# winddori2002/DEX-TTS

Hardware: AMD Instinct MI355X
Metric: mel-frames/s at n_timesteps=50, 80-ch mel (sampler only); RTF (higher is better)
Workload: dtype bf16; 1 GPU; gedex_b1: gedex_lj B=1/GPU T=512 n_timesteps=50 (BASELINE.json configs[1]); global_batch=1, frames=512, hipgraph=False, parallelism=1 GPU

## Files before the change

dex_tts_amd/csrc/conv3x3_bf16.hip:

```cpp
#include "kernels.h"
#include <cstdlib>
#include <cstdio>
#include "lp_util.h"
#include "kernels_lp.h"
#include "conv_gn.h"

namespace dex {
namespace DEX_LP_NS {

typedef float f32x16 __attribute__((ext_vector_type(16)));
typedef unsigned short u16;
typedef unsigned u32x4 __attribute__((ext_vector_type(4)));

__device__ __forceinline__ float cv_mish(float x) {
    const float e = __expf(fminf(x, 20.f));
    const float n = e * (e + 2.f);
    return x * (n * __builtin_amdgcn_rcpf(n + 2.f));
}

template <int NT, int COUT>
__device__ __forceinline__ void cv_epilogue(const Conv3P& p, f32x16 (&acc)[NT], int b, int ho, int w0, int nbase, int lane, int tid,
                                            long long* gnred) {
    const int i = lane & 31, hh = lane >> 5;
    constexpr int cpg = COUT / 8;
    if (p.gn_stats) { if (tid < 16) gnred[tid] = 0; __syncthreads(); }
    const bool full = ho < p.H && w0 + 32 <= p.W;
    const long ybase = (long)b * p.H * p.W * COUT + ((long)ho * p.W + w0 + 4 * hh) * COUT + nbase + i;
    float* yl = p.Y + ybase;
    u16* yh = reinterpret_cast<u16*>(p.Y) + ybase;
    const bool yb = p.y_bf16 != 0;
#pragma unroll
    for (int t = 0; t < NT; ++t) {
        const int n = nbase + t * 32 + i;
        const float bias = p.bias[n];
        float gs = 0.f, gss = 0.f;
        if (full && yb) {
            const bool odd = (lane & 1) != 0;
            u16* yp = yh + (odd ? 16 * COUT - 1 : 0) + t * 32;
#pragma unroll
            for (int r = 0; r < 16; ++r) { const float v = acc[t][r] + bias; gs += v; gss = fmaf(v, v, gss); }
#pragma unroll
            for (int j = 0; j < 8; ++j) {
                const float lo_r = acc[t][j] + bias, hi_r = acc[t][8 + j] + bias;
                const float recv = lane_xor1(odd ? lo_r : hi_r);
                const float mine = odd ? hi_r : lo_r;
                const unsigned pk = odd ? pack2_lp(recv, mine) : pack2_lp(mine, recv);
                *reinterpret_cast<unsigned*>(yp + ((j & 3) + 8 * (j >> 2)) * COUT) = pk;
            }
        } else if (full) {
            const bool odd = (lane & 1) != 0;
            float* yp = yl + (odd ? 16 * COUT - 1 : 0) + t * 32;
#pragma unroll
            for (int r = 0; r < 16; ++r) { const float v = acc[t][r] + bias; gs += v; gss = fmaf(v, v, gss); }
#pragma unroll
            for (int j = 0; j < 8; ++j) {
                const float lo_r = acc[t][j] + bias, hi_r = acc[t][8 + j] + bias;
                const float recv = lane_xor1(odd ? lo_r : hi_r);
                const float mine = odd ? hi_r : lo_r;
                *reinterpret_cast<float2*>(yp + ((j & 3) + 8 * (j >> 2)) * COUT) = odd ? make_float2(recv, mine) : make_float2(mine, recv);
            }
        } else {
#pragma unroll
            for (int r = 0; r < 16; ++r) {
                const int wo = w0 + (r & 3) + 8 * (r >> 2) + 4 * hh;
                const bool ok = ho < p.H && wo < p.W;
                const float v = acc[t][r] + bias;
                const float vs = ok ? v : 0.f;
                gs += vs; gss = fmaf(vs, vs, gss);
                if (ok) {
                    if (yb) yh[((r & 3) + 8 * (r >> 2)) * COUT + t * 32] = lp_bits(v);
                    else yl[((r & 3) + 8 * (r >> 2)) * COUT + t * 32] = v;
                }
            }
        }
        if (p.gn_stats) {
            for (int o = 1; o < cpg; o <<= 1) { gs += __shfl_xor(gs, o); gss += __shfl_xor(gss, o); }
            gs += __shfl_xor(gs, 32); gss += __shfl_xor(gss, 32);
            if (hh == 0 && (i & (cpg - 1)) == 0) {
                const double inv_n = 1.0 / ((double)p.H * p.W * cpg);
                gn_add(&gnred[(n / cpg) * 2], gn_fix(gs, inv_n)); gn_add(&gnred[(n / cpg) * 2 + 1], gn_fix(gss, inv_n));
            }
        }
    }
    if (p.gn_stats) {
        __syncthreads();
        if (tid < 16) {
            const long long v = gnred[tid];
            if (v != 0) {
                const int slot = (blockIdx.x + blockIdx.y * gridDim.x) % GN_SLOTS;
                gn_add(p.gn_stats + (((long)b * 8 + (tid >> 1)) * GN_SLOTS + slot) * 2 + (tid & 1), v);
            }
        }
    }
}

template <int NT, int COUT>
__device__ __forceinline__ void cv_res_store(const Conv3P& p, const f32x16 (&accr)[NT], int b, int ho, int w0, int nb, int lane) {
    const int i = lane & 31, hh = lane >> 5;
    float* yl = p.res_y + ((long)b * p.H * p.W + (long)ho * p.W + w0 + 4 * hh) * COUT + nb + i;
    const bool rfull = ho < p.H && w0 + 32 <= p.W;
    const bool odd = (lane & 1) != 0;
#pragma unroll
    for (int t = 0; t < NT; ++t) {
        const float bias = p.res_b[nb + t * 32 + i];
        if (rfull) {
            float* yp = yl + (odd ? 16 * COUT - 1 : 0) + t * 32;
#pragma unroll
            for (int j = 0; j < 8; ++j) {
                const float lo_r = accr[t][j] + bias, hi_r = accr[t][8 + j] + bias;
                const float recv = lane_xor1(odd ? lo_r : hi_r);
                const float mine = odd ? hi_r : lo_r;
                *reinterpret_cast<float2*>(yp + ((j & 3) + 8 * (j >> 2)) * COUT) = odd ? make_float2(recv, mine) : make_float2(mine, recv);
            }
        } else {
#pragma unroll
            for (int r = 0; r < 16; ++r) {
                const int wo = w0 + (r & 3) + 8 * (r >> 2) + 4 * hh;
                if (ho < p.H && wo < p.W) yl[((r & 3) + 8 * (r >> 2)) * COUT + t * 32] = accr[t][r] + bias;
            }
        }
    }
}

template <int CC, int COUT, int NSL, int TH, bool PRO2 = false, bool RES = false, bool XB = false, int NW = 4, bool RW = false>
__global__ __launch_bounds__(64 * NW) void conv3x3_lp_kernel(const Conv3P p) {
    constexpr int PW = 34, PH = TH + 2;
    constexpr int LDP = CC + 8;
    constexpr int WN = NW / TH;
    constexpr int NTHR = 64 * NW;
    constexpr int NT = NSL / 32 / WN;
    constexpr int NSLICE = COUT / NSL;
    constexpr int ITEMS = PH * PW * (CC / 8);
    constexpr int NI = (ITEMS + NTHR - 1) / NTHR;
    constexpr int WITEMS = NSL * CC / 8;
    constexpr int WPT = (WITEMS + NTHR - 1) / NTHR;
    constexpr bool WFULL = WITEMS % NTHR == 0;
    constexpr int RING = CC == 128 ? (PRO2 ? 1 : 2) : 3;
    constexpr int NPASS = RW ? 1
                        : TH == 5 ? (CC == 128 ? (PRO2 ? 6 : 3) : (PRO2 ? 3 : XB ? 1 : 2))
                                  : CC == 128 ? (TH == 8 ? (PRO2 ? 8 : 4) : (PRO2 ? 5 : 2)) : (PRO2 ? 3 : 1);
    constexpr int NIP = (NI + NPASS - 1) / NPASS;
    constexpr int RWI = 9 * WITEMS;
    constexpr int RWPT = (RWI + NTHR - 1) / NTHR;
    constexpr int RWB = (RWPT + NPASS - 1) / NPASS;
#ifdef DEX_LP_WSPLIT
    constexpr int NTAP = 18;
#else
    constexpr int NTAP = 9;
#endif
    static_assert(NT >= 1 && WPT >= 1 && NW % TH == 0 && NTHR % (CC / 8) == 0, "tile");
    static_assert(!RW || NTAP == 9, "the resident schedule holds nine taps");
    extern __shared__ __attribute__((aligned(16))) u16 smem[];
    u16* patch = smem;
    u16* wbuf = smem + PH * PW * LDP;
    u16* rbuf = wbuf + (RW ? 9 : 2) * NSL * LDP;
    __shared__ long long gnred[16];
    constexpr int COEF_N = (TH == 8) ? 128 : 256;
    __shared__ __attribute__((aligned(16))) float coef[3][COEF_N];

    const int tid = threadIdx.x, lane = tid & 63, wave = tid >> 6;
    const int i = lane & 31, hh = lane >> 5;
    const int wrow = wave % TH, wcol = wave / TH;
#ifdef DEX_TIMING
    long long tk[8] = {0, 0, 0, 0, 0, 0, 0, 0};
    const long long tk0 = __builtin_readcyclecounter();
    long long tlast = tk0;
#define CSTAMP(k) do { const long long now_ = __builtin_readcyclecounter(); tk[k] += now_ - tlast; tlast = now_; } while (0)
#else
#define CSTAMP(k) do {} while (0)
#endif
    const int xs = p.skip_dead ? (int)((blockIdx.x + blockIdx.y + blockIdx.z) % gridDim.x) : (int)blockIdx.x;
    const int w0 = xs * 32, h0 = blockIdx.y * TH;
    const int b = blockIdx.z / NSLICE, slice = blockIdx.z % NSLICE;
    const int step = p.step + b * p.row_bstride;
    const float* X = p.X + (long)b * p.H * p.W * p.ldx + p.x_coff;
    const u16* Xh = reinterpret_cast<const u16*>(p.X) + (long)b * p.H * p.W * p.ldx + p.x_coff;
    const float* mrow = p.mask + (long)b * p.mask_bstride;
    const int K = 9 * p.Cin;
    const u16* Wg = reinterpret_cast<const u16*>(p.Wbf) + (long)slice * NSL * K;
    const bool pro = p.pro_stats != nullptr;
    if constexpr (!PRO2) {
        if (p.skip_dead) {
            const int wi = w0 - 1 + (lane < 34 ? lane : 33);
            const float mv = (unsigned)wi < (unsigned)p.W ? mrow[wi * p.mask_ws] : 0.f;
            if (__builtin_amdgcn_ballot_w64(mv != 0.f) == 0) {
                f32x16 zacc[NT];
#pragma unroll
                for (int t = 0; t < NT; ++t)
#pragma unroll
                    for (int r = 0; r < 16; ++r) zacc[t][r] = 0.f;
                if constexpr (RES) cv_res_store<NT, COUT>(p, zacc, b, h0 + wrow, w0, slice * NSL + wcol * NT * 32, lane);
                cv_epilogue<NT, COUT>(p, zacc, b, h0 + wrow, w0, slice * NSL + wcol * NT * 32, lane, tid, gnred);
                return;
            }
        }
    }

    f32x16 acc[NT];
#pragma unroll
    for (int t = 0; t < NT; ++t)
#pragma unroll
        for (int r = 0; r < 16; ++r) acc[t][r] = 0.f;

    f32x16 accr[RES ? NT : 1];
    if constexpr (RES) {
#pragma unroll
        for (int t = 0; t < NT; ++t)
#pragma unroll
            for (int r = 0; r < 16; ++r) accr[t][r] = 0.f;
    }
    int wofs[WPT], wlds[WPT];
    bool wok[WPT];
#pragma unroll
    for (int j = 0; j < WPT; ++j) {
        const int it = tid + NTHR * j;
        const int n = it / (CC / 8), c8 = (it % (CC / 8)) * 8;
        wofs[j] = n * K + c8;
        wlds[j] = n * LDP + c8;
        wok[j] = WFULL || it < WITEMS;
    }
    const int pc8 = (tid % (CC / 8)) * 8;

    CvGnLoads gnl{};
    if (pro) gnl = cv_gn_issue(p, b, tid, step);
    const int nchunk = RW ? 1 : p.Cin / CC;
    for (int ch = 0; ch < nchunk; ++ch) {
        const int cbase = ch * CC;
        u32x4 w0r[WPT], wr[RING][WPT], rwr[RES ? WPT : 1];
#ifdef DEX_LP_WSPLIT
        u32x4 rwl[RES ? WPT : 1];
#define WS_TAPOFS(t) ((long)((t) % 9) * p.Cin + ((t) >= 9 ? p.w_lo_off : 0L))
#else
#define WS_TAPOFS(t) ((long)(t) * p.Cin)
#endif
        float4 sc0, sc1, sh0, sh1, t0, t1;
#pragma unroll
        for (int ps = 0; ps < NPASS; ++ps) {
            float4 pf0[NIP], pf1[XB ? 1 : NIP], rf0[PRO2 ? NIP : 1], rf1[PRO2 ? NIP : 1];
            float pmk[NIP];
            bool pin[NIP];
#pragma unroll
            for (int q = 0; q < NIP; ++q) {
                const int it = min(tid + NTHR * (ps * NIP + q), ITEMS - 1);
                const int px = it / (CC / 8);
                const int pw = px % PW, ph = px / PW;
                const int hi = h0 + ph - 1, wi = w0 + pw - 1;
                const bool inb = (unsigned)hi < (unsigned)p.H && (unsigned)wi < (unsigned)p.W;
                const int hc = inb ? hi : 0, wc = inb ? wi : 0;
                if constexpr (XB) {
                    pf0[q] = *reinterpret_cast<const float4*>(Xh + ((long)hc * p.W + wc) * p.ldx + cbase + pc8);
                } else {
                    const float* src = X + ((long)hc * p.W + wc) * p.ldx + cbase + pc8;
                    pf0[q] = *reinterpret_cast<const float4*>(src);
                    pf1[q] = *reinterpret_cast<const float4*>(src + 4);
                }
                if constexpr (PRO2) {
                    const float* rs = p.pro_res + ((long)b * p.H * p.W + (long)hc * p.W + wc) * p.Cin + cbase + pc8;
                    rf0[q] = *reinterpret_cast<const float4*>(rs);
                    rf1[q] = *reinterpret_cast<const float4*>(rs + 4);
                }
                const float mk = mrow[wc * p.mask_ws];
                pmk[q] = inb ? mk : 0.f;
                pin[q] = inb;
            }
            u32x4 rwv[RW ? RWB : 1];
            if constexpr (RW) {
#pragma unroll
                for (int j = 0; j < RWB; ++j) {
                    const int it = tid + NTHR * (ps * RWB + j);
                    if (ps * RWB + j < RWPT && (RWI % NTHR == 0 || it < RWI)) {
                        const int r = it % WITEMS;
                        rwv[j] = *reinterpret_cast<const u32x4*>(Wg + (r / (CC / 8)) * K + (it / WITEMS) * p.Cin + (r % (CC / 8)) * 8);
                    }
                }
            }
            if (ps == 0) {
                if constexpr (RES) {
                    const u16* Rg = reinterpret_cast<const u16*>(p.res_w) + (long)slice * NSL * p.Cin;
#pragma unroll
                    for (int j = 0; j < WPT; ++j) {
                        const int it = tid + NTHR * j;
                        if (!wok[j]) continue;
                        rwr[j] = *reinterpret_cast<const u32x4*>(Rg + (long)(it / (CC / 8)) * p.Cin + cbase + (it % (CC / 8)) * 8);
#ifdef DEX_LP_WSPLIT
                        rwl[j] = *reinterpret_cast<const u32x4*>(Rg + p.res_lo_off + (long)(it / (CC / 8)) * p.Cin + cbase + (it % (CC / 8)) * 8);
#endif
                    }
                }
                if constexpr (!RW) {
#pragma unroll
                    for (int j = 0; j < WPT; ++j) if (wok[j]) w0r[j] = *reinterpret_cast<const u32x4*>(Wg + wofs[j] + cbase);
#pragma unroll
                    for (int s = 0; s < RING; ++s)
#pragma unroll
                        for (int j = 0; j < WPT; ++j) if (wok[j]) wr[s][j] = *reinterpret_cast<const u32x4*>(Wg + wofs[j] + WS_TAPOFS(s + 1) + cbase);
                }
                CSTAMP(0);
                if (pro && ch == 0) cv_gn_finish<COEF_N>(p, gnl, tid, coef);
                __builtin_amdgcn_sched_barrier(0);
                if (!RW || pro) lds_barrier();
                CSTAMP(1);
                if (pro) {
                    const int c = cbase + pc8;
                    sc0 = *reinterpret_cast<const float4*>(&coef[0][c]); sc1 = *reinterpret_cast<const float4*>(&coef[0][c + 4]);
                    sh0 = *reinterpret_cast<const float4*>(&coef[1][c]); sh1 = *reinterpret_cast<const float4*>(&coef[1][c + 4]);
                    t0 = *reinterpret_cast<const float4*>(&coef[2][c]); t1 = *reinterpret_cast<const float4*>(&coef[2][c + 4]);
                }
            }
#pragma unroll
            for (int q = 0; q < NIP; ++q) {
                float4 f0, f1;
                if constexpr (XB) {
                    const float4 r = pf0[q];
                    const unsigned u0 = __float_as_uint(r.x), u1 = __float_as_uint(r.y), u2 = __float_as_uint(r.z), u3 = __float_as_uint(r.w);
                    f0 = make_float4(lp_lo(u0), lp_hi(u0), lp_lo(u1), lp_hi(u1));
                    f1 = make_float4(lp_lo(u2), lp_hi(u2), lp_lo(u3), lp_hi(u3));
                } else { f0 = pf0[q]; f1 = pf1[q]; }
#ifdef DEX_SCALAR_PROLOGUE
                if (pro) {
                    f0.x = cv_mish(fmaf(f0.x, sc0.x, sh0.x)) + t0.x; f0.y = cv_mish(fmaf(f0.y, sc0.y, sh0.y)) + t0.y;
                    f0.z = cv_mish(fmaf(f0.z, sc0.z, sh0.z)) + t0.z; f0.w = cv_mish(fmaf(f0.w, sc0.w, sh0.w)) + t0.w;
                    f1.x = cv_mish(fmaf(f1.x, sc1.x, sh1.x)) + t1.x; f1.y = cv_mish(fmaf(f1.y, sc1.y, sh1.y)) + t1.y;
                    f1.z = cv_mish(fmaf(f1.z, sc1.z, sh1.z)) + t1.z; f1.w = cv_mish(fmaf(f1.w, sc1.w, sh1.w)) + t1.w;
                }
#else
                if (pro) {
                    const f32x2 a0 = mish2_add(f32x2{f0.x, f0.y} * f32x2{sc0.x, sc0.y} + f32x2{sh0.x, sh0.y}, f32x2{t0.x, t0.y});
                    const f32x2 a1 = mish2_add(f32x2{f0.z, f0.w} * f32x2{sc0.z, sc0.w} + f32x2{sh0.z, sh0.w}, f32x2{t0.z, t0.w});
                    const f32x2 a2 = mish2_add(f32x2{f1.x, f1.y} * f32x2{sc1.x, sc1.y} + f32x2{sh1.x, sh1.y}, f32x2{t1.x, t1.y});
                    const f32x2 a3 = mish2_add(f32x2{f1.z, f1.w} * f32x2{sc1.z, sc1.w} + f32x2{sh1.z, sh1.w}, f32x2{t1.z, t1.w});
                    f0 = make_float4(a0.x, a0.y, a1.x, a1.y); f1 = make_float4(a2.x, a2.y, a3.x, a3.y);
                }
#endif
                const float mk = pmk[q];
                const int it = tid + NTHR * (ps * NIP + q);
                if constexpr (PRO2) {
                    f0.x = fmaf(f0.x, mk, rf0[q].x); f0.y = fmaf(f0.y, mk, rf0[q].y); f0.z = fmaf(f0.z, mk, rf0[q].z); f0.w = fmaf(f0.w, mk, rf0[q].w);
                    f1.x = fmaf(f1.x, mk, rf1[q].x); f1.y = fmaf(f1.y, mk, rf1[q].y); f1.z = fmaf(f1.z, mk, rf1[q].z); f1.w = fmaf(f1.w, mk, rf1[q].w);
                    const int px_ = it / (CC / 8), pw_ = px_ % PW, ph_ = px_ / PW;
                    if (slice == 0 && it < ITEMS && pin[q] && ph_ >= 1 && ph_ <= TH && pw_ >= 1 && pw_ <= 32) {
                        float* xo = p.pro_xout + ((long)b * p.H * p.W + (long)(h0 + ph_ - 1) * p.W + (w0 + pw_ - 1)) * p.Cin + cbase + pc8;
                        *reinterpret_cast<float4*>(xo) = f0;
                        *reinterpret_cast<float4*>(xo + 4) = f1;
                    }
                }
                uint4 v;
                v.x = pack2_lp(f0.x * mk, f0.y * mk); v.y = pack2_lp(f0.z * mk, f0.w * mk);
                v.z = pack2_lp(f1.x * mk, f1.y * mk); v.w = pack2_lp(f1.z * mk, f1.w * mk);
                if (it < ITEMS) *reinterpret_cast<uint4*>(patch + (it / (CC / 8)) * LDP + pc8) = v;
            }
            if constexpr (RW) {
#pragma unroll
                for (int j = 0; j < RWB; ++j) {
                    const int it = tid + NTHR * (ps * RWB + j);
                    if (ps * RWB + j < RWPT && (RWI % NTHR == 0 || it < RWI)) {
                        const int r = it % WITEMS;
                        *reinterpret_cast<u32x4*>(wbuf + ((it / WITEMS) * NSL + r / (CC / 8)) * LDP + (r % (CC / 8)) * 8) = rwv[j];
                    }
                }
            }
        }
        if constexpr (!RW) {
#pragma unroll
            for (int j = 0; j < WPT; ++j) if (wok[j]) *reinterpret_cast<u32x4*>(wbuf + wlds[j]) = w0r[j];
        }
        if constexpr (RES) {
#pragma unroll
            for (int j = 0; j < WPT; ++j) if (wok[j]) *reinterpret_cast<u32x4*>(rbuf + wlds[j]) = rwr[j];
        }
        CSTAMP(2);
        if constexpr (RW) {
            lds_barrier();
            constexpr int KS = CC / 16;
            const u16* ap = patch + (wrow * PW + i) * LDP + hh * 8;
            const u16* bp = wbuf + (wcol * NT * 32 + i) * LDP + hh * 8;
            const u16* rp = rbuf + (wcol * NT * 32 + i) * LDP + hh * 8;
            lp8 af[2], bf[2][NT], rf[2][RES ? NT : 1];
            af[0] = *reinterpret_cast<const lp8*>(ap);
#pragma unroll
            for (int t = 0; t < NT; ++t) bf[0][t] = *reinterpret_cast<const lp8*>(bp + t * 32 * LDP);
#pragma unroll
            for (int s = 0; s < 9 * KS; ++s) {
                if (s + 1 < 9 * KS) {
                    const int tap = (s + 1) / KS, ks = (s + 1) % KS, kh = tap / 3, kw = tap - kh * 3;
                    af[(s + 1) & 1] = *reinterpret_cast<const lp8*>(ap + (kh * PW + kw) * LDP + ks * 16);
#pragma unroll
                    for (int t = 0; t < NT; ++t) bf[(s + 1) & 1][t] = *reinterpret_cast<const lp8*>(bp + (tap * NSL + t * 32) * LDP + ks * 16);
                    if constexpr (RES) {
                        if (tap == 4) {
#pragma unroll
                            for (int t = 0; t < NT; ++t) rf[(s + 1) & 1][t] = *reinterpret_cast<const lp8*>(rp + t * 32 * LDP + ks * 16);
                        }
                    }
                }
                __builtin_amdgcn_sched_barrier(0);
#pragma unroll
                for (int t = 0; t < NT; ++t) acc[t] = DEX_MFMA_LP(af[s & 1], bf[s & 1][t], acc[t], 0, 0, 0);
                if constexpr (RES) {
                    if (s / KS == 4) {
#pragma unroll
                        for (int t = 0; t < NT; ++t) accr[t] = DEX_MFMA_LP(af[s & 1], rf[s & 1][t], accr[t], 0, 0, 0);
                    }
                }
                __builtin_amdgcn_sched_barrier(0);
            }
        } else {
#pragma unroll
        for (int tt = 0; tt < NTAP; ++tt) {
            const int tap = tt % 9;
            lds_barrier();
            if (tt + 1 < NTAP) {
                u16* wn = wbuf + ((tt + 1) & 1) * NSL * LDP;
#pragma unroll
                for (int j = 0; j < WPT; ++j) if (wok[j]) *reinterpret_cast<u32x4*>(wn + wlds[j]) = wr[tt % RING][j];
                if (tt + 1 + RING < NTAP) {
#pragma unroll
                    for (int j = 0; j < WPT; ++j)
                        if (wok[j]) wr[tt % RING][j] = *reinterpret_cast<const u32x4*>(Wg + wofs[j] + WS_TAPOFS(tt + 1 + RING) + cbase);
                }
                __builtin_amdgcn_sched_barrier(0);
            }
#ifdef DEX_LP_WSPLIT
            if constexpr (RES) {
                if (tt == 5) {
#pragma unroll
                    for (int j = 0; j < WPT; ++j) if (wok[j]) *reinterpret_cast<u32x4*>(rbuf + wlds[j]) = rwl[j];
                }
            }
#endif
            const u16* wb = wbuf + (tt & 1) * NSL * LDP;
            const int kh = tap / 3, kw = tap - kh * 3;
            const u16* ap = patch + ((wrow + kh) * PW + i + kw) * LDP + hh * 8;
            const u16* bp = wb + (wcol * NT * 32 + i) * LDP + hh * 8;
#pragma unroll
            for (int ks = 0; ks < CC / 16; ++ks) {
                const lp8 af = *reinterpret_cast<const lp8*>(ap + ks * 16);
#pragma unroll
                for (int t = 0; t < NT; ++t) {
                    const lp8 bf = *reinterpret_cast<const lp8*>(bp + t * 32 * LDP + ks * 16);
                    acc[t] = DEX_MFMA_LP(af, bf, acc[t], 0, 0, 0);
                }
                if constexpr (RES) {
                    if (tap == 4) {
#pragma unroll
                        for (int t = 0; t < NT; ++t) {
                            const lp8 rf = *reinterpret_cast<const lp8*>(rbuf + (wcol * NT * 32 + t * 32 + i) * LDP + hh * 8 + ks * 16);
                            accr[t] = DEX_MFMA_LP(af, rf, accr[t], 0, 0, 0);
                        }
                    }
                }
            }
        }
        }
    }
    if constexpr (RES) cv_res_store<NT, COUT>(p, accr, b, h0 + wrow, w0, slice * NSL + wcol * NT * 32, lane);
    CSTAMP(3);
    cv_epilogue<NT, COUT>(p, acc, b, h0 + wrow, w0, slice * NSL + wcol * NT * 32, lane, tid, gnred);
#ifdef DEX_TIMING
    CSTAMP(4);
    if (p.dbg && tid == 0) {
        long long* d = p.dbg + ((long)(blockIdx.z * gridDim.y + blockIdx.y) * gridDim.x + blockIdx.x) * 8;
        for (int k = 0; k < 5; ++k) d[k] = tk[k];
        unsigned hw, xcc;
        asm volatile("s_getreg_b32 %0, hwreg(HW_REG_HW_ID)" : "=s"(hw));
        asm volatile("s_getreg_b32 %0, hwreg(HW_REG_XCC_ID)" : "=s"(xcc));
        d[5] = hw; d[6] = xcc & 15u;
        d[7] = __builtin_readcyclecounter() - tk0;
    }
#endif
}

template <int CC, int COUT, int NSL, int TH, bool PRO2 = false, bool RES = false, bool XB = false, int NW = 4, bool RW = false>
static void launch_c3(const Conv3P& p, hipStream_t st) {
    constexpr int LDP = CC + 8;
    const size_t lds = ((size_t)(TH + 2) * 34 * LDP + ((RW ? 9 : 2) + (RES ? 1 : 0)) * NSL * LDP) * sizeof(u16);
    static bool attr = false;
    if (!attr) {
        hipFuncSetAttribute(reinterpret_cast<const void*>(&conv3x3_lp_kernel<CC, COUT, NSL, TH, PRO2, RES, XB, NW, RW>), hipFuncAttributeMaxDynamicSharedMemorySize, (int)lds);
        attr = true;
    }
    dim3 grid((p.W + 31) / 32, (p.H + TH - 1) / TH, p.B * (COUT / NSL));
    if (RW && p.Cin != CC) { fprintf(stderr, "libdexamd: resident conv3x3 form needs Cin == %d in one chunk (got %d)\n", CC, p.Cin); abort(); }
    Conv3P q = p;
    q.skip_dead = (p.B >= 4 && (long)grid.x * grid.y * grid.z >= 1024 && knob_or("DEX_CONV_SKIP_DEAD", 1) != 0) ? 1 : 0;
    static char sym[96];
    if (!sym[0]) snprintf(sym, sizeof sym, "conv3x3_lp_kernel<%d,%d,%d,%d,%d,%d,%d,%d%s>", CC, COUT, NSL, TH, (int)PRO2, (int)RES, (int)XB, NW, RW ? ",resident" : "");
    g_last_symbol = sym;
    hipLaunchKernelGGL((conv3x3_lp_kernel<CC, COUT, NSL, TH, PRO2, RES, XB, NW, RW>), grid, dim3(64 * NW), lds, st, q);
}

bool conv3x3_bf16_tail_supported(int C) {
#if defined(DEX_LP_WSPLIT) && !defined(DEX_WS_HAVE_CONV3)
    return false;
#endif
    return C == 64 || C == 128; }
bool conv3x3_bf16_xb_supported(int Cin, int Cout) {
#if defined(DEX_LP_WSPLIT) && !defined(DEX_WS_HAVE_CONV3)
    return false;
#endif
    return Cin == Cout && (Cin == 64 || Cin == 128); }
bool conv3x3_bf16_res_supported(int Cin, int Cout) {
#if defined(DEX_LP_WSPLIT) && !defined(DEX_WS_HAVE_CONV3_RES)
    return false;
#endif
    return (Cout == 128 && Cin == 64) || (Cout == 64 && (Cin == 128 || Cin == 256)); }
bool conv3x3_bf16_supported(int Cin, int Cout) {
#if defined(DEX_LP_WSPLIT) && !defined(DEX_WS_HAVE_CONV3)
    return false;
#endif
   
    return (Cin == 64 || Cin == 128 || Cin == 256) && (Cout == 64 || Cout == 128);
}

bool conv3x3_plain_lp_in_supported(int H, int W, int B, int Cin, int Cout) {
#if defined(DEX_LP_WSPLIT) && !defined(DEX_WS_HAVE_CONV3)
    return false;
#endif
   
    const int w8 = knob_or("DEX_CONV_W8", 1);
    const long tiles4 = (long)((W + 31) / 32) * ((H + 3) / 4) * B;
    return w8 && tiles4 >= 256 && Cin == 64 && Cout == 128;
}

bool conv3x3_cat_lp_in_supported(int H, int W, int B, int Cin, int Cout) {
#if defined(DEX_LP_WSPLIT) && !defined(DEX_WS_HAVE_CONV3_RES)
    return false;
#endif
   
    if (Cout != 64 || Cin < 128 || Cin % 128 != 0) return false;
    const int w8 = knob_or("DEX_CONV_W8", 1);
    const long small_max = knob_or("DEX_CONV_SMALL_MAX", 256);
    const long tiles4 = (long)((W + 31) / 32) * ((H + 3) / 4) * B;
    return w8 && tiles4 >= small_max;
}

static bool conv3x3_resident_on() { return knob_or("DEX_CONV_RESIDENT", 1) != 0; }

static bool launch_c3_round1(const Conv3P& p, bool small, hipStream_t st) {
    if (!knob_or("DEX_CONV_ROUND1", 1)) return false;
    const bool tail_ = p.pro_res != nullptr;
#ifdef DEX_LP_WSPLIT
    const bool c64 = p.Cin == 64 && p.Cout == 64 && !p.res_w && !tail_;
#else
    const bool c64 = p.Cin == 64 && p.Cout == 64 && !p.res_w;
#endif
    const bool r128 = p.Cin == 64 && p.Cout == 128 && p.res_w && !tail_ && !p.x_bf16;
    if (!c64 && !r128) return false;
    const long strips = (long)((p.W + 31) / 32) * p.B;
    const long cur = c64 ? strips * (small ? (p.H + 1) / 2 : (p.H + 3) / 4) : strips * (small ? (p.H + 1) / 2 * 2 : (p.H + 3) / 4);
    const long one = strips * ((p.H + 4) / 5) * (c64 ? 1 : 4);
    const long ncu = device_cus();
    if (cur <= ncu || one > ncu || one * 4 < ncu * 3) return false;
#ifndef DEX_LP_WSPLIT
    if (conv3x3_resident_on()) {
        if (c64 && !tail_) {
            p.x_bf16 ? launch_c3<64, 64, 64, 5, false, false, true, 10, true>(p, st) : launch_c3<64, 64, 64, 5, false, false, false, 10, true>(p, st);
            return true;
        }
        if (!c64) { launch_c3<64, 128, 32, 5, false, true, false, 5, true>(p, st); return true; }
    }
#endif
    if (c64) {
#ifndef DEX_LP_WSPLIT
        if (tail_) { p.x_bf16 ? launch_c3<64, 64, 64, 5, true, false, true, 10>(p, st) : launch_c3<64, 64, 64, 5, true, false, false, 10>(p, st); return true; }
#endif
        p.x_bf16 ? launch_c3<64, 64, 64, 5, false, false, true, 10>(p, st) : launch_c3<64, 64, 64, 5, false, false, false, 10>(p, st);
    } else {
        launch_c3<64, 128, 32, 5, false, true, false, 5>(p, st);
    }
    return true;
}

static bool launch_c3_small_resident(const Conv3P& p, bool small, hipStream_t st) {
#ifdef DEX_LP_WSPLIT
    return false;
#else
    if (!small || !conv3x3_resident_on() || p.Cin != 64 || p.Cout != 64 || p.res_w) return false;
    if ((long)((p.W + 31) / 32) * ((p.H + 1) / 2) * p.B > device_cus()) return false;
    const bool tail_ = p.pro_res != nullptr;
    if (tail_) { p.x_bf16 ? launch_c3<64, 64, 64, 2, true, false, true, 4, true>(p, st) : launch_c3<64, 64, 64, 2, true, false, false, 4, true>(p, st); }
    else { p.x_bf16 ? launch_c3<64, 64, 64, 2, false, false, true, 4, true>(p, st) : launch_c3<64, 64, 64, 2, false, false, false, 4, true>(p, st); }
    return true;
#endif
}

void launch_conv3x3_lp(const Conv3P& p, hipStream_t st) {
    if (const int tpw = conv3x3_stream_tiles(p)) { launch_conv3x3_stream(p, tpw, st); return; }
    if (conv3x3_regw_form(p)) { launch_conv3x3_regw(p, st); return; }
    const bool tail_ = p.pro_res != nullptr;
    const long tiles4 = (long)((p.W + 31) / 32) * ((p.H + 3) / 4) * p.B;
    const long small_max = knob_or("DEX_CONV_SMALL_MAX", 256);
    const bool small = tiles4 < small_max;
    const int w8 = knob_or("DEX_CONV_W8", 1);
    const int th8 = knob_or("DEX_CONV_TH8", 1);
    if (th8 && w8 && !small && !tail_ && p.Cin == 128 && p.Cout == 128 && !p.res_w && p.H % 8 == 0 && (long)((p.W + 31) / 32) * (p.H / 8) * p.B >= 512) {
        p.x_bf16 ? launch_c3<128, 128, 128, 8, false, false, true, 8>(p, st) : launch_c3<128, 128, 128, 8, false, false, false, 8>(p, st);
        return;
    }
    if (w8 && !small && p.Cin == 128 && p.Cout == 128 && !p.res_w) {
        if (p.x_bf16) { tail_ ? launch_c3<128, 128, 128, 4, true, false, true, 8>(p, st) : launch_c3<128, 128, 128, 4, false, false, true, 8>(p, st); }
        else { tail_ ? launch_c3<128, 128, 128, 4, true, false, false, 8>(p, st) : launch_c3<128, 128, 128, 4, false, false, false, 8>(p, st); }
        return;
    }
    if (w8 && !small && p.res_w && p.Cout == 128 && p.Cin == 64) {
        p.x_bf16 ? launch_c3<64, 128, 128, 4, false, true, true, 8>(p, st) : launch_c3<64, 128, 128, 4, false, true, false, 8>(p, st);
        return;
    }
    if (th8 && w8 && !small && p.res_w && p.Cout == 64 && p.Cin >= 128 && !p.pro_stats && p.H % 8 == 0 && (long)((p.W + 31) / 32) * (p.H / 8) * p.B >= 512) {
        p.x_bf16 ? launch_c3<128, 64, 64, 8, false, true, true, 8>(p, st) : launch_c3<128, 64, 64, 8, false, true, false, 8>(p, st);
        return;
    }
    if (w8 && !small && p.res_w && p.Cout == 64 && p.Cin >= 128) {
        p.x_bf16 ? launch_c3<128, 64, 64, 4, false, true, true, 8>(p, st) : launch_c3<128, 64, 64, 4, false, true, false, 8>(p, st);
        return;
    }
    if (launch_c3_round1(p, small, st)) return;
    if (launch_c3_small_resident(p, small, st)) return;
    if (p.x_bf16) {
        if (tail_) {
            if (p.Cin == 64) { small ? launch_c3<64, 64, 64, 2, true, false, true>(p, st) : launch_c3<64, 64, 64, 4, true, false, true>(p, st); }
            else { small ? launch_c3<128, 128, 64, 2, true, false, true>(p, st) : launch_c3<128, 128, 128, 4, true, false, true>(p, st); }
        } else {
            if (p.Cin == 64) { small ? launch_c3<64, 64, 64, 2, false, false, true>(p, st) : launch_c3<64, 64, 64, 4, false, false, true>(p, st); }
            else { small ? launch_c3<128, 128, 64, 2, false, false, true>(p, st) : launch_c3<128, 128, 128, 4, false, false, true>(p, st); }
        }
        return;
    }
    if (tail_) {
        if (p.Cin == 64 && p.Cout == 64) { small ? launch_c3<64, 64, 64, 2, true>(p, st) : launch_c3<64, 64, 64, 4, true>(p, st); }
        else { small ? launch_c3<128, 128, 64, 2, true>(p, st) : launch_c3<128, 128, 128, 4, true>(p, st); }
        return;
    }
    if (p.res_w) {
        if (p.Cout == 128 && p.Cin == 64) { small ? launch_c3<64, 128, 64, 2, false, true>(p, st) : launch_c3<64, 128, 128, 4, false, true>(p, st); return; }
        if (p.Cout == 64 && p.Cin >= 128) { small ? launch_c3<128, 64, 64, 2, false, true>(p, st) : launch_c3<128, 64, 64, 4, false, true>(p, st); return; }
    }
    if (p.Cout == 64) {
        if (p.Cin == 64) { small ? launch_c3<64, 64, 64, 2>(p, st) : launch_c3<64, 64, 64, 4>(p, st); }
        else { small ? launch_c3<128, 64, 64, 2>(p, st) : launch_c3<128, 64, 64, 4>(p, st); }
    } else {
        if (p.Cin == 64) { small ? launch_c3<64, 128, 64, 2>(p, st) : launch_c3<64, 128, 128, 4>(p, st); }
        else { small ? launch_c3<128, 128, 64, 2>(p, st) : launch_c3<128, 128, 128, 4>(p, st); }
    }
}

}
}
```

dex_tts_amd/csrc/dex_api.hip:

```cpp
#include <hip/hip_runtime.h>
#include <cstdlib>

#include <cmath>
#include <cstdarg>
#include <atomic>
#include <cstdio>
#include <mutex>
#include <cstring>
#include <map>
#include <unordered_map>
#include <string_view>
#include <string>
#include <vector>

#include "../../include/dex_amd.h"
#include "kernels.h"
#include "weight_store.h"

using namespace dex;

namespace dex {
namespace {
const char* const KNOB_NAMES[] = {
    "DEX_CONV_STREAM", "DEX_CONV_PP", "DEX_CONV_SKIP_DEAD", "DEX_H_BF16", "DEX_ATTN_SEPARATE", "DEX_ATTN_Q64", "DEX_ATTN_Q64_TAIL", "DEX_ATTN_Q64_HALF", "DEX_DIT_XCDS", "DEX_ATTN_GENERIC", "DEX_RES2", "DEX_LP_INTER", "DEX_DIT_CHAIN",
    "DEX_DIT_CLUSTER", "DEX_DIT_CLUSTER_LOCAL", "DEX_ATTN_X_LP", "DEX_RES_X_LP", "DEX_CAT_LP", "DEX_XCD_MAP", "DEX_DEBUG_DROP_HANDOFF", "DEX_PATCH_FUSED",
    "DEX_CONV_DOWN", "DEX_CONVT_UP", "DEX_DEBUG_PLAN",
    "DEX_ATTN_SHARED_W8", "DEX_CONVT_MT", "DEX_CONVT_WGS", "DEX_CONV_DOWN_WGS", "DEX_CONV_REGW", "DEX_CONV_REGW_RES", "DEX_CONV_SMALL_MAX", "DEX_CONV_TH8",
    "DEX_CONV_W8", "DEX_DWCONV_CAP", "DEX_FINAL_CAP", "DEX_FIRST_CAP", "DEX_FIRST_MFMA", "DEX_GEMM_NWALK", "DEX_NWALK_SPLIT", "DEX_NWALK_BM", "DEX_POS_COL", "DEX_POS_COL_MIN",
    "DEX_POS_CT", "DEX_REGW_MIN_TILES", "DEX_REGW_WGS", "DEX_ROWCHAIN64", "DEX_ROWCHAIN64A", "DEX_TIV_CAP", "DEX_TV_CHAIN", "DEX_TIV_FOLD", "DEX_LINATTN_NSUB", "DEX_TV_FOLD", "DEX_OUT2_MIN", "DEX_NWALK_DMA",
    "DEX_LINATTN_HEADWAVES", "DEX_LINATTN_OUT2_HW", "DEX_CONV_ROUND1", "DEX_CONV_RESIDENT", "DEX_KVCTX_ROWS", "DEX_OUT2_ROWS", "DEX_PE_TOK", "DEX_NWALK_SMALL"};
constexpr int N_KNOBS = (int)(sizeof(KNOB_NAMES) / sizeof(KNOB_NAMES[0]));
int knob_parse(const char* e) {
    if (!e) return KNOB_UNSET;
    char* end = nullptr;
    const long v = strtol(e, &end, 10);
    if (end == e) {
        static bool warned = false;
        if (!warned) { warned = true; fprintf(stderr, "libdexamd: ignoring a DEX_* knob whose value '%s' is not an integer\n", e); }
        return KNOB_UNSET;
    }
    return (int)v;
}
struct KnobSnapshot {
    int v[N_KNOBS];
    KnobSnapshot() { for (int i = 0; i < N_KNOBS; ++i) v[i] = knob_parse(getenv(KNOB_NAMES[i])); }
};
thread_local const KnobSnapshot* t_knobs = nullptr;
struct WsplitScope {
    bool prev;
    explicit WsplitScope(bool on) : prev(g_lp_wsplit) { g_lp_wsplit = on; }
    ~WsplitScope() { g_lp_wsplit = prev; }
};
struct KnobScope {
    const KnobSnapshot* prev;
    explicit KnobScope(const KnobSnapshot* k) : prev(t_knobs) { t_knobs = k; }
    ~KnobScope() { t_knobs = prev; }
};
}
static int knob_index(const char* name) {
    static const std::unordered_map<std::string_view, int> idx = [] {
        std::unordered_map<std::string_view, int> m;
        for (int i = 0; i < N_KNOBS; ++i) m.emplace(KNOB_NAMES[i], i);
        return m;
    }();
    const auto it = idx.find(std::string_view(name));
    return it == idx.end() ? -1 : it->second;
}
int knob(const char* name) {
    if (t_knobs) {
        const int i = knob_index(name);
        if (i >= 0) return t_knobs->v[i];
    }
    return knob_parse(getenv(name));
}
}
static_assert(PREC_FP32 == DEX_PREC_FP32 && PREC_BF16 == DEX_PREC_BF16 && PREC_FP16 == DEX_PREC_FP16 && PREC_FP16X2 == DEX_PREC_FP16X2, "kernels.h mirrors DexPrecision");

namespace {
void xcd_map_probe();

struct TD { float* p; int ld; int coff; int C; int lp = 0; };

struct ResW { PackedW w1, w2, wr; const float *b1, *g1, *be1, *b2, *g2, *be2, *br, *mlp_w, *mlp_b; int cin, cout; };
constexpr int ATT_KSPLIT_MAX = 4;
static int att_split_cap(long tokens) { return tokens <= 20480 ? 8 : ATT_KSPLIT_MAX; }
static bool attention_q64_regime(int N, int B) {
    if (N < 1024) return dit_sep64_small_n(N, B) && dit_rowchain64_form(N, B, 0);
    const int ks = attention_q64_ksplit(N, B, att_split_cap((long)B * N));
    const int nt32 = (N + 31) / 32, ng = (nt32 + 7) / 8;
    return 2L * B * ng * ks >= 128;
}
struct LinW { PackedW wqkv; const float *wqkv_raw, *wout_raw, *bias_eff, *g; LpView wkv[3], wq_frag[3]; int C; };
struct DitBlockW { PackedW wqkv, wproj, wfc1, wfc2; const float *bqkv, *bproj, *bfc1, *bfc2, *ada_w, *ada_b; };

struct Prof { std::string name; hipEvent_t a, b; double flops, bytes; };
struct ProfAgg { std::string name; int calls; double ms, flops, bytes; };

struct Arena {
    char* base = nullptr; size_t off = 0, cap = 0; bool dry = true;
    void* take(size_t bytes) {
        off = (off + 255) & ~size_t(255);
        void* p = dry ? nullptr : (void*)(base + off);
        if (!dry && trace) fprintf(stderr, "plan[%d] off %zu bytes %zu\n", trace++, off, bytes);
        off += bytes;
        return p;
    }
    int trace = 0;
    float* f(size_t n) { return (float*)take(n * sizeof(float)); }
};

}

struct DexCtx : WeightStore {
    DexCtx() : WeightStore("") {}
    DexConfig cfg{};
    int lpi() const { return precision == DEX_PREC_FP16X2 ? 2 : precision == DEX_PREC_FP16 ? 1 : 0; }
    int lp_kind() const { return precision == DEX_PREC_BF16 ? 1 : 2; }
    bool lp() const { return precision != DEX_PREC_FP32; }
    bool tuned = true;
    int precision = DEX_PREC_FP32;
    std::vector<std::vector<ResW>> down_res, up_res;
    std::vector<LinW> down_lin, up_lin;
    std::vector<PackedW> down_ds_w;
    std::vector<std::vector<PackedW>> up_us_w;
    std::vector<const float*> down_ds_b, up_us_b;
    const float *fc_w3 = nullptr, *fc_w1 = nullptr;
    PackedW fin_w, pe_pw, fl_w, tv_wk, tv_wv, tv_wl;
    PackedW pos_w;
    const float *fin_b = nullptr, *fin_g = nullptr, *fin_be = nullptr, *fconv_w = nullptr, *fconv_b = nullptr;
    const float *pe_dw = nullptr, *pe_db = nullptr, *pe_pb = nullptr, *pos_b = nullptr, *freq_pos = nullptr;
    std::vector<DitBlockW> blocks;
    const float *fl_b = nullptr, *fl_ada_w = nullptr, *fl_ada_b = nullptr;
    const float *tv_wq_raw = nullptr;
    float *mel_basis = nullptr, *mel_filt = nullptr; void* mel_ws = nullptr; size_t mel_ws_bytes = 0;
    const int* last_xerr = nullptr;
    int* st_host = nullptr; hipEvent_t st_ev = nullptr; bool st_pending = false;
    struct Tap { std::string name; const float* p; std::vector<int64_t> shape; };
    std::vector<Tap> taps;
    bool prof_on = false;
    std::vector<Prof> prof;
    std::vector<ProfAgg> prof_agg;
    struct GraphEntry { std::vector<uint64_t> key; hipGraphExec_t exec; uint64_t stamp; const int* xerr; };
    std::vector<GraphEntry> graphs;
    uint64_t graph_clock = 0;
    void drop_graphs() { for (auto& g : graphs) hipGraphExecDestroy(g.exec); graphs.clear(); }
    template <typename F> int replay(const std::vector<uint64_t>& key, hipStream_t st, F&& enqueue);
    void reset_records() {
        taps.clear();
        if (prof_on) { for (auto& pr : prof) { hipEventDestroy(pr.a); hipEventDestroy(pr.b); } prof.clear(); prof_agg.clear(); }
    }
};

template <typename F> int DexCtx::replay(const std::vector<uint64_t>& key, hipStream_t st, F&& enqueue) {
    GraphEntry* hit = nullptr;
    for (auto& g : graphs) if (g.key == key) { hit = &g; break; }
    if (!hit) {
        constexpr size_t MAX_GRAPHS = 8;
        if (graphs.size() >= MAX_GRAPHS) {
            size_t lru = 0;
            for (size_t i = 1; i < graphs.size(); ++i) if (graphs[i].stamp < graphs[lru].stamp) lru = i;
            hipGraphExecDestroy(graphs[lru].exec);
            graphs.erase(graphs.begin() + lru);
        }
        hipGraph_t graph = nullptr;
        DEX_HIPCHK(this, hipStreamBeginCapture(st, hipStreamCaptureModeThreadLocal));
        const int rc = enqueue();
        hipError_t ec = hipStreamEndCapture(st, &graph);
        if (rc) { if (graph) hipGraphDestroy(graph); return rc; }
        if (ec != hipSuccess || !graph) return fail(DEX_ERR_HIP, "stream capture failed: %s", hipGetErrorString(ec));
        hipGraphExec_t exec = nullptr;
        ec = hipGraphInstantiate(&exec, graph, nullptr, nullptr, 0);
        hipGraphDestroy(graph);
        if (ec != hipSuccess) return fail(DEX_ERR_HIP, "hipGraphInstantiate failed: %s", hipGetErrorString(ec));
        graphs.push_back({key, exec, 0, last_xerr});
        hit = &graphs.back();
    }
    last_xerr = hit->xerr;
    hit->stamp = ++graph_clock;
    DEX_HIPCHK(this, hipGraphLaunch(hit->exec, st));
    DEX_HIPCHK(this, hipGetLastError());
    return DEX_OK;
}

// ... 1758 lines not shown
```

Baseline: 29540 mel-frames/s.

## Prefetch next pass of conv3x3 patch items while staging current pass

Adds an SR template mode for the 128-channel, TH=2, small conv3x3 kernel. In this mode each patch item's global loads for the next pass are issued right after the current item is consumed, under scheduling barriers, instead of all loads for a pass being issued at the start of that pass. This is meant to hide load latency across passes. The PRO2 tail output store also becomes an unconditional buffer store whose out-of-range offset is dropped by the hardware, which removes the branch. It is on by default for the small-grid path via the DEX_CONV_STAGE_RING knob; it keeps more registers live and could lower occupancy.

Result: no change. 29690 mel-frames/s, median of 6 (+0.5%).

```diff
diff --git a/dex_tts_amd/csrc/conv3x3_bf16.hip b/dex_tts_amd/csrc/conv3x3_bf16.hip
--- a/dex_tts_amd/csrc/conv3x3_bf16.hip
+++ b/dex_tts_amd/csrc/conv3x3_bf16.hip
@@ -122,7 +122,34 @@
     }
 }
 
-template <int CC, int COUT, int NSL, int TH, bool PRO2 = false, bool RES = false, bool XB = false, int NW = 4, bool RW = false>
+template <int CC, int TH, bool PRO2, bool XB>
+__device__ __forceinline__ void cv_request(const Conv3P& p, const float* X, const u16* Xh, const float* mrow, int b, int h0, int w0, int cofs,
+                                           int it, float4& a0, float4& a1, float4& r0, float4& r1, float& mk, bool& in) {
+    constexpr int PW = 34;
+    it = min(it, (TH + 2) * PW * (CC / 8) - 1);
+    const int px = it / (CC / 8);
+    const int pw = px % PW, ph = px / PW;
+    const int hi = h0 + ph - 1, wi = w0 + pw - 1;
+    const bool inb = (unsigned)hi < (unsigned)p.H && (unsigned)wi < (unsigned)p.W;
+    const int hc = inb ? hi : 0, wc = inb ? wi : 0;
+    if constexpr (XB) {
+        a0 = *reinterpret_cast<const float4*>(Xh + ((long)hc * p.W + wc) * p.ldx + cofs);
+    } else {
+        const float* src = X + ((long)hc * p.W + wc) * p.ldx + cofs;
+        a0 = *reinterpret_cast<const float4*>(src);
+        a1 = *reinterpret_cast<const float4*>(src + 4);
+    }
+    if constexpr (PRO2) {
+        const float* rs = p.pro_res + ((long)b * p.H * p.W + (long)hc * p.W + wc) * p.Cin + cofs;
+        r0 = *reinterpret_cast<const float4*>(rs);
+        r1 = *reinterpret_cast<const float4*>(rs + 4);
+    }
+    const float m = mrow[wc * p.mask_ws];
+    mk = inb ? m : 0.f;
+    in = inb;
+}
+
+template <int CC, int COUT, int NSL, int TH, bool PRO2 = false, bool RES = false, bool XB = false, int NW = 4, bool RW = false, bool SR = false>
 __global__ __launch_bounds__(64 * NW) void conv3x3_lp_kernel(const Conv3P p) {
     constexpr int PW = 34, PH = TH + 2;
     constexpr int LDP = CC + 8;
@@ -150,6 +177,7 @@
 #endif
     static_assert(NT >= 1 && WPT >= 1 && NW % TH == 0 && NTHR % (CC / 8) == 0, "tile");
     static_assert(!RW || NTAP == 9, "the resident schedule holds nine taps");
+    static_assert(!SR || (!RW && NPASS > 1), "the item ring replaces the passes of a streamed form that has several");
     extern __shared__ __attribute__((aligned(16))) u16 smem[];
     u16* patch = smem;
     u16* wbuf = smem + PH * PW * LDP;
@@ -221,6 +249,9 @@
     }
     const int pc8 = (tid % (CC / 8)) * 8;
 
+    const __amdgpu_buffer_rsrc_t xo_rsrc = __builtin_amdgcn_make_buffer_rsrc(
+        const_cast<float*>(PRO2 && SR ? p.pro_xout + (long)b * p.H * p.W * p.Cin : p.bias), 0,
+        PRO2 && SR && slice == 0 ? (unsigned)((long)p.H * p.W * p.Cin * 4) : 0u, 0x00020000);
     CvGnLoads gnl{};
     if (pro) gnl = cv_gn_issue(p, b, tid, step);
     const int nchunk = RW ? 1 : p.Cin / CC;
@@ -234,11 +265,19 @@
 #define WS_TAPOFS(t) ((long)(t) * p.Cin)
 #endif
         float4 sc0, sc1, sh0, sh1, t0, t1;
+        float4 pf0[NIP], pf1[XB ? 1 : NIP], rf0[PRO2 ? NIP : 1], rf1[PRO2 ? NIP : 1];
+        float pmk[NIP];
+        bool pin[NIP];
 #pragma unroll
         for (int ps = 0; ps < NPASS; ++ps) {
-            float4 pf0[NIP], pf1[XB ? 1 : NIP], rf0[PRO2 ? NIP : 1], rf1[PRO2 ? NIP : 1];
-            float pmk[NIP];
-            bool pin[NIP];
+            if constexpr (SR) {
+                if (ps == 0) {
+#pragma unroll
+                    for (int q = 0; q < NIP; ++q)
+                        cv_request<CC, TH, PRO2, XB>(p, X, Xh, mrow, b, h0, w0, cbase + pc8, tid + NTHR * q, pf0[q], pf1[XB ? 0 : q],
+                                                     rf0[PRO2 ? q : 0], rf1[PRO2 ? q : 0], pmk[q], pin[q]);
+                }
+            } else {
 #pragma unroll
             for (int q = 0; q < NIP; ++q) {
                 const int it = min(tid + NTHR * (ps * NIP + q), ITEMS - 1);
@@ -263,6 +302,7 @@
                 pmk[q] = inb ? mk : 0.f;
                 pin[q] = inb;
             }
+            }
             u32x4 rwv[RW ? RWB : 1];
             if constexpr (RW) {
 #pragma unroll
@@ -309,6 +349,7 @@
             }
 #pragma unroll
             for (int q = 0; q < NIP; ++q) {
+                if (SR && ps * NIP + q >= NI) continue;
                 float4 f0, f1;
                 if constexpr (XB) {
                     const float4 r = pf0[q];
@@ -333,10 +374,28 @@
                 }
 #endif
                 const float mk = pmk[q];
+                bool inq = false;
+                if constexpr (SR) inq = pin[q];
                 const int it = tid + NTHR * (ps * NIP + q);
                 if constexpr (PRO2) {
                     f0.x = fmaf(f0.x, mk, rf0[q].x); f0.y = fmaf(f0.y, mk, rf0[q].y); f0.z = fmaf(f0.z, mk, rf0[q].z); f0.w = fmaf(f0.w, mk, rf0[q].w);
                     f1.x = fmaf(f1.x, mk, rf1[q].x); f1.y = fmaf(f1.y, mk, rf1[q].y); f1.z = fmaf(f1.z, mk, rf1[q].z); f1.w = fmaf(f1.w, mk, rf1[q].w);
+                }
+                if constexpr (SR) {
+                    if (ps + 1 < NPASS && (ps + 1) * NIP + q < NI) {
+                        __builtin_amdgcn_sched_barrier(0);
+                        cv_request<CC, TH, PRO2, XB>(p, X, Xh, mrow, b, h0, w0, cbase + pc8, tid + NTHR * ((ps + 1) * NIP + q), pf0[q],
+                                                     pf1[XB ? 0 : q], rf0[PRO2 ? q : 0], rf1[PRO2 ? q : 0], pmk[q], pin[q]);
+                        __builtin_amdgcn_sched_barrier(0);
+                    }
+                }
+                if constexpr (PRO2 && SR) {
+                    const int px_ = it / (CC / 8), pw_ = px_ % PW, ph_ = px_ / PW;
+                    const bool own = it < ITEMS && inq && ph_ >= 1 && ph_ <= TH && pw_ >= 1 && pw_ <= 32;
+                    const unsigned off = own ? (unsigned)((((h0 + ph_ - 1) * p.W + (w0 + pw_ - 1)) * p.Cin + cbase + pc8) * 4) : 0x80000000u;
+                    __builtin_amdgcn_raw_buffer_store_b128(u32x4{__float_as_uint(f0.x), __float_as_uint(f0.y), __float_as_uint(f0.z), __float_as_uint(f0.w)}, xo_rsrc, off, 0, 0);
+                    __builtin_amdgcn_raw_buffer_store_b128(u32x4{__float_as_uint(f1.x), __float_as_uint(f1.y), __float_as_uint(f1.z), __float_as_uint(f1.w)}, xo_rsrc, off + 16u, 0, 0);
+                } else if constexpr (PRO2) {
                     const int px_ = it / (CC / 8), pw_ = px_ % PW, ph_ = px_ / PW;
                     if (slice == 0 && it < ITEMS && pin[q] && ph_ >= 1 && ph_ <= TH && pw_ >= 1 && pw_ <= 32) {
                         float* xo = p.pro_xout + ((long)b * p.H * p.W + (long)(h0 + ph_ - 1) * p.W + (w0 + pw_ - 1)) * p.Cin + cbase + pc8;
@@ -470,13 +529,17 @@
 #endif
 }
 
-template <int CC, int COUT, int NSL, int TH, bool PRO2 = false, bool RES = false, bool XB = false, int NW = 4, bool RW = false>
+constexpr bool cv_stage_ring_form(int CC, int COUT, int TH, bool RES, int NW, bool RW) {
+    return CC == 128 && COUT == 128 && TH == 2 && NW == 4 && !RW && !RES;
+}
+
+template <int CC, int COUT, int NSL, int TH, bool PRO2 = false, bool RES = false, bool XB = false, int NW = 4, bool RW = false, bool SR = false>
 static void launch_c3(const Conv3P& p, hipStream_t st) {
     constexpr int LDP = CC + 8;
     const size_t lds = ((size_t)(TH + 2) * 34 * LDP + ((RW ? 9 : 2) + (RES ? 1 : 0)) * NSL * LDP) * sizeof(u16);
     static bool attr = false;
     if (!attr) {
-        hipFuncSetAttribute(reinterpret_cast<const void*>(&conv3x3_lp_kernel<CC, COUT, NSL, TH, PRO2, RES, XB, NW, RW>), hipFuncAttributeMaxDynamicSharedMemorySize, (int)lds);
+        hipFuncSetAttribute(reinterpret_cast<const void*>(&conv3x3_lp_kernel<CC, COUT, NSL, TH, PRO2, RES, XB, NW, RW, SR>), hipFuncAttributeMaxDynamicSharedMemorySize, (int)lds);
         attr = true;
     }
     dim3 grid((p.W + 31) / 32, (p.H + TH - 1) / TH, p.B * (COUT / NSL));
@@ -484,9 +547,18 @@
     Conv3P q = p;
     q.skip_dead = (p.B >= 4 && (long)grid.x * grid.y * grid.z >= 1024 && knob_or("DEX_CONV_SKIP_DEAD", 1) != 0) ? 1 : 0;
     static char sym[96];
-    if (!sym[0]) snprintf(sym, sizeof sym, "conv3x3_lp_kernel<%d,%d,%d,%d,%d,%d,%d,%d%s>", CC, COUT, NSL, TH, (int)PRO2, (int)RES, (int)XB, NW, RW ? ",resident" : "");
+    constexpr bool passes = !SR && cv_stage_ring_form(CC, COUT, TH, RES, NW, RW);
+    if (!sym[0]) snprintf(sym, sizeof sym, "conv3x3_lp_kernel<%d,%d,%d,%d,%d,%d,%d,%d%s>", CC, COUT, NSL, TH, (int)PRO2, (int)RES, (int)XB, NW, RW ? ",resident" : passes ? ",passes" : "");
     g_last_symbol = sym;
-    hipLaunchKernelGGL((conv3x3_lp_kernel<CC, COUT, NSL, TH, PRO2, RES, XB, NW, RW>), grid, dim3(64 * NW), lds, st, q);
+    hipLaunchKernelGGL((conv3x3_lp_kernel<CC, COUT, NSL, TH, PRO2, RES, XB, NW, RW, SR>), grid, dim3(64 * NW), lds, st, q);
+}
+
+template <int CC, int COUT, int NSL, int TH, bool PRO2 = false, bool RES = false, bool XB = false>
+static void launch_c3_staged(const Conv3P& p, hipStream_t st) {
+    static_assert(cv_stage_ring_form(CC, COUT, TH, RES, 4, false), "no ring schedule of this form");
+    const bool fits = !PRO2 || (long)p.H * p.W * p.Cin * 4 < (1L << 31);
+    if (fits && knob_or("DEX_CONV_STAGE_RING", 1) != 0) launch_c3<CC, COUT, NSL, TH, PRO2, RES, XB, 4, false, true>(p, st);
+    else launch_c3<CC, COUT, NSL, TH, PRO2, RES, XB, 4, false, false>(p, st);
 }
 
 bool conv3x3_bf16_tail_supported(int C) {
@@ -619,16 +691,16 @@
     if (p.x_bf16) {
         if (tail_) {
             if (p.Cin == 64) { small ? launch_c3<64, 64, 64, 2, true, false, true>(p, st) : launch_c3<64, 64, 64, 4, true, false, true>(p, st); }
-            else { small ? launch_c3<128, 128, 64, 2, true, false, true>(p, st) : launch_c3<128, 128, 128, 4, true, false, true>(p, st); }
+            else { small ? launch_c3_staged<128, 128, 64, 2, true, false, true>(p, st) : launch_c3<128, 128, 128, 4, true, false, true>(p, st); }
         } else {
             if (p.Cin == 64) { small ? launch_c3<64, 64, 64, 2, false, false, true>(p, st) : launch_c3<64, 64, 64, 4, false, false, true>(p, st); }
-            else { small ? launch_c3<128, 128, 64, 2, false, false, true>(p, st) : launch_c3<128, 128, 128, 4, false, false, true>(p, st); }
+            else { small ? launch_c3_staged<128, 128, 64, 2, false, false, true>(p, st) : launch_c3<128, 128, 128, 4, false, false, true>(p, st); }
         }
         return;
     }
     if (tail_) {
         if (p.Cin == 64 && p.Cout == 64) { small ? launch_c3<64, 64, 64, 2, true>(p, st) : launch_c3<64, 64, 64, 4, true>(p, st); }
-        else { small ? launch_c3<128, 128, 64, 2, true>(p, st) : launch_c3<128, 128, 128, 4, true>(p, st); }
+        else { small ? launch_c3_staged<128, 128, 64, 2, true>(p, st) : launch_c3<128, 128, 128, 4, true>(p, st); }
         return;
     }
     if (p.res_w) {
@@ -640,9 +712,9 @@
         else { small ? launch_c3<128, 64, 64, 2>(p, st) : launch_c3<128, 64, 64, 4>(p, st); }
     } else {
         if (p.Cin == 64) { small ? launch_c3<64, 128, 64, 2>(p, st) : launch_c3<64, 128, 128, 4>(p, st); }
-        else { small ? launch_c3<128, 128, 64, 2>(p, st) : launch_c3<128, 128, 128, 4>(p, st); }
-    }
-}
-
-}
-}
+        else { small ? launch_c3_staged<128, 128, 64, 2>(p, st) : launch_c3<128, 128, 128, 4>(p, st); }
+    }
+}
+
+}
+}
diff --git a/dex_tts_amd/csrc/dex_api.hip b/dex_tts_amd/csrc/dex_api.hip
--- a/dex_tts_amd/csrc/dex_api.hip
+++ b/dex_tts_amd/csrc/dex_api.hip
@@ -28,7 +28,7 @@
     "DEX_ATTN_SHARED_W8", "DEX_CONVT_MT", "DEX_CONVT_WGS", "DEX_CONV_DOWN_WGS", "DEX_CONV_REGW", "DEX_CONV_REGW_RES", "DEX_CONV_SMALL_MAX", "DEX_CONV_TH8",
     "DEX_CONV_W8", "DEX_DWCONV_CAP", "DEX_FINAL_CAP", "DEX_FIRST_CAP", "DEX_FIRST_MFMA", "DEX_GEMM_NWALK", "DEX_NWALK_SPLIT", "DEX_NWALK_BM", "DEX_POS_COL", "DEX_POS_COL_MIN",
     "DEX_POS_CT", "DEX_REGW_MIN_TILES", "DEX_REGW_WGS", "DEX_ROWCHAIN64", "DEX_ROWCHAIN64A", "DEX_TIV_CAP", "DEX_TV_CHAIN", "DEX_TIV_FOLD", "DEX_LINATTN_NSUB", "DEX_TV_FOLD", "DEX_OUT2_MIN", "DEX_NWALK_DMA",
-    "DEX_LINATTN_HEADWAVES", "DEX_LINATTN_OUT2_HW", "DEX_CONV_ROUND1", "DEX_CONV_RESIDENT", "DEX_KVCTX_ROWS", "DEX_OUT2_ROWS", "DEX_PE_TOK", "DEX_NWALK_SMALL"};
+    "DEX_LINATTN_HEADWAVES", "DEX_LINATTN_OUT2_HW", "DEX_CONV_ROUND1", "DEX_CONV_RESIDENT", "DEX_KVCTX_ROWS", "DEX_OUT2_ROWS", "DEX_PE_TOK", "DEX_NWALK_SMALL", "DEX_CONV_STAGE_RING"};
 constexpr int N_KNOBS = (int)(sizeof(KNOB_NAMES) / sizeof(KNOB_NAMES[0]));
 int knob_parse(const char* e) {
     if (!e) return KNOB_UNSET;
```
